# NIRVANALAN/LN3Diff

Measured on NVIDIA H100. Metric: denoised-latents/sec, higher is better.
Workload: dtype bf16

## Files before the change

ln3diff_b200/csrc/attention_wgmma.cu:

```cuda
#include <cstdlib>

#include "common.cuh"
#include "ln3_internal.h"

namespace ln3 {

static constexpr int kQT = 128;
static constexpr int kKT = 128;
static constexpr int kSW = 64;
static constexpr int kTileBytes = 128 * kSW * 2;
static constexpr int kStages = 4;
static constexpr int kThreads = 2 * 128 + 32;
static constexpr int kOrderBar = 1;
static constexpr int kTail = 8;
static constexpr int kTailBytes = 128 * kTail * 2;
static constexpr int kTailSmem = 2 * kTailBytes + kStages * 3 * kTailBytes;
template <int HD>
static constexpr int kFmhaSmem = 1024 + kTileBytes * (1 + 2 * kStages) + (HD > kSW ? kTailSmem : 0) + 256;

template <int HD>
struct FmhaTailMaps {
  CUtensorMap q, k, v;
};
template <>
struct FmhaTailMaps<64> {};

struct FmhaParams {
  int Lq, Lkv, Lkv2;
  int nb1, nb2;
  int H, n_qt;
  long long n_tiles;
  float scale_log2;
  int causal;
  __nv_bfloat16* out;
  long long o_ld, o_bs;
};

struct Tile {
  int q0, h, b, nb1, nblocks;
};

__device__ __forceinline__ Tile decode_tile(const FmhaParams& p, long long t) {
  Tile d;
  const long long bh = t / p.n_qt;
  d.q0 = static_cast<int>(t - bh * p.n_qt) * kQT;
  d.h = static_cast<int>(bh % p.H);
  d.b = static_cast<int>(bh / p.H);
  d.nb1 = p.causal ? min(p.nb1, (min(d.q0 + kQT, p.Lq) - 1) / kKT + 1) : p.nb1;
  d.nblocks = d.nb1 + p.nb2;
  return d;
}

__device__ __forceinline__ void softmax_block(const FmhaParams& p, float* s, float* m_run, float* l_run,
                                              float* alpha, int j, int nb1, int r0, int q) {
  const bool second = j >= nb1;
  const int kbase = (second ? j - nb1 : j) * kKT;
  const int klen = second ? p.Lkv2 : p.Lkv;
  const bool need_mask = kbase + kKT > klen || (p.causal && !second && kbase + kKT - 1 > r0);
  float mx[2] = {-INFINITY, -INFINITY};
#pragma unroll
  for (int i = 0; i < kKT / 8; ++i) {
#pragma unroll
    for (int e = 0; e < 4; ++e) {
      float v = __fmul_rn(s[4 * i + e], p.scale_log2);
      if (need_mask) {
        const int key = kbase + 8 * i + 2 * q + (e & 1);
        const int row = r0 + 8 * (e >> 1);
        if (key >= klen || (p.causal && !second && key > row)) v = -INFINITY;
      }
      s[4 * i + e] = v;
      mx[e >> 1] = fmaxf(mx[e >> 1], v);
    }
  }
  float m_use[2];
#pragma unroll
  for (int r = 0; r < 2; ++r) {
    mx[r] = fmaxf(mx[r], __shfl_xor_sync(0xffffffffu, mx[r], 1));
    mx[r] = fmaxf(mx[r], __shfl_xor_sync(0xffffffffu, mx[r], 2));
    const float m_new = fmaxf(m_run[r], mx[r]);
    m_use[r] = m_new == -INFINITY ? 0.f : m_new;
    alpha[r] = fast_exp2(__fsub_rn(m_run[r], m_use[r]));
    m_run[r] = m_new;
  }
#pragma unroll
  for (int kk = 0; kk < kKT / 16; ++kk) {
#pragma unroll
    for (int t = 0; t < 8; ++t) {
      const int r = (t >> 1) & 1;
      const float e = fast_exp2(__fsub_rn(s[8 * kk + t], m_use[r]));
      s[8 * kk + t] = e;
      l_run[r] = (kk == 0 && (t == 0 || t == 2)) ? __fmaf_rn(alpha[r], l_run[r], e) : __fadd_rn(l_run[r], e);
    }
  }
}

__device__ __forceinline__ void pack_p(const float* s, uint32_t (*pa)[4]) {
#pragma unroll
  for (int kk = 0; kk < kKT / 16; ++kk) {
    pa[kk][0] = pack_bf16x2(s[8 * kk + 0], s[8 * kk + 1]);
    pa[kk][1] = pack_bf16x2(s[8 * kk + 2], s[8 * kk + 3]);
    pa[kk][2] = pack_bf16x2(s[8 * kk + 4], s[8 * kk + 5]);
    pa[kk][3] = pack_bf16x2(s[8 * kk + 6], s[8 * kk + 7]);
  }
}

template <int HD>
__device__ __forceinline__ void issue_s(float* s, uint64_t q_desc, uint64_t k_desc, uint64_t qt_desc, uint64_t kt_desc) {
#pragma unroll
  for (int k = 0; k < kSW / 16; ++k) wgmma_m64n128k16_ss(s, q_desc + 2 * k, k_desc + 2 * k, k != 0 ? 1u : 0u);
  if constexpr (HD > kSW) wgmma_m64n128k16_ss(s, qt_desc, kt_desc, 1u);
  wgmma_commit();
}

template <int HD>
__device__ __forceinline__ void issue_pv(float* o, float* ot, const uint32_t (*pa)[4], uint64_t v_desc,
                                         uint64_t vt_desc) {
#pragma unroll
  for (int kk = 0; kk < kKT / 16; ++kk) {
    wgmma_m64n64k16_rs_tb(o, pa[kk], v_desc + kk * 128, 1u);
    if constexpr (HD > kSW) wgmma_m64n8k16_rs_tb(ot, pa[kk], vt_desc + kk * ((16 * kTail * 2) >> 4), 1u);
  }
  wgmma_commit();
}

template <int HD>
__global__ void __launch_bounds__(kThreads, 1)
fmha_fwd_kernel(const __grid_constant__ CUtensorMap tmap_q, const __grid_constant__ CUtensorMap tmap_k,
                const __grid_constant__ CUtensorMap tmap_v, const __grid_constant__ CUtensorMap tmap_k2,
                const __grid_constant__ CUtensorMap tmap_v2, const FmhaParams p,
                const __grid_constant__ FmhaTailMaps<HD> tails) {
  constexpr bool kHasTail = HD > kSW;
  extern __shared__ uint8_t smem_raw[];
  uint8_t* smem = reinterpret_cast<uint8_t*>((reinterpret_cast<uintptr_t>(smem_raw) + 1023) &
                                             ~static_cast<uintptr_t>(1023));
  uint8_t* sQ = smem;
  uint8_t* sK = sQ + kTileBytes;
  uint8_t* sV = sK + kStages * kTileBytes;
  uint8_t* sQt = sV + kStages * kTileBytes;
  uint8_t* sKt = sQt + 2 * kTailBytes;
  uint8_t* sVt = sKt + kStages * 2 * kTailBytes;
  uint64_t* bars = reinterpret_cast<uint64_t*>(sV + kStages * kTileBytes + (kHasTail ? kTailSmem : 0));
  uint64_t* q_full = bars;
  uint64_t* q_empty = bars + 1;
  uint64_t* kv_full = bars + 2;
  uint64_t* kv_empty = bars + 2 + kStages;

  const int warp = threadIdx.x >> 5;
  const int lane = threadIdx.x & 31;

  if (threadIdx.x == 0) {
    tma_prefetch_desc(&tmap_q);
    tma_prefetch_desc(&tmap_k);
    tma_prefetch_desc(&tmap_v);
    mbar_init(q_full, 1);
    mbar_init(q_empty, 2);
    for (int i = 0; i < kStages; ++i) {
      mbar_init(&kv_full[i], 1);
      mbar_init(&kv_empty[i], 2);
    }
    fence_barrier_init();
  }
  if constexpr (kHasTail) {
    for (int i = threadIdx.x; i < (1 + kStages) * (kTailBytes / 16); i += kThreads) {
      const int tile = i / (kTailBytes / 16), off = (i % (kTailBytes / 16)) * 16;
      *reinterpret_cast<uint4*>(sQt + tile * 2 * kTailBytes + kTailBytes + off) = make_uint4(0, 0, 0, 0);
    }
    fence_proxy_async_smem();
  }
  __syncthreads();

  if (warp == 8) {
    if (lane == 0) {
      int stage = 0;
      uint32_t phase = 0, tcount = 0;
      for (long long t = blockIdx.x; t < p.n_tiles; t += gridDim.x, ++tcount) {
        const Tile d = decode_tile(p, t);
        mbar_wait_silent(q_empty, (tcount & 1) ^ 1);
        mbar_arrive_expect_tx(q_full, kTileBytes + (kHasTail ? kTailBytes : 0));
        tma_load_3d(sQ, &tmap_q, q_full, d.h * HD, d.q0, d.b);
        if constexpr (kHasTail) tma_load_3d(sQt, &tails.q, q_full, d.h * HD + kSW, d.q0, d.b);
        for (int j = 0; j < d.nblocks; ++j) {
          mbar_wait_silent(&kv_empty[stage], phase ^ 1);
          mbar_arrive_expect_tx(&kv_full[stage], 2 * kTileBytes + (kHasTail ? 2 * kTailBytes : 0));
          const bool second = j >= d.nb1;
          const int row = (second ? j - d.nb1 : j) * kKT;
          tma_load_3d(sK + stage * kTileBytes, second ? &tmap_k2 : &tmap_k, &kv_full[stage], d.h * HD, row, d.b);
          tma_load_3d(sV + stage * kTileBytes, second ? &tmap_v2 : &tmap_v, &kv_full[stage], d.h * HD, row, d.b);
          if constexpr (kHasTail) {
            tma_load_3d(sKt + stage * 2 * kTailBytes, &tails.k, &kv_full[stage], d.h * HD + kSW, row, d.b);
            tma_load_3d(sVt + stage * kTailBytes, &tails.v, &kv_full[stage], d.h * HD + kSW, row, d.b);
          }
          if (++stage == kStages) {
            stage = 0;
            phase ^= 1;
          }
        }
      }
    }
    return;
  }

  const int wg = warp >> 2;
  const int g = lane >> 2, q = lane & 3;
  const bool leader = (threadIdx.x & 127) == 0;
  const uint64_t q_desc = make_smem_desc_sw128(smem_u32(sQ + wg * (64 * 128)), 16, 1024);
  const uint64_t k_desc0 = make_smem_desc_sw128(smem_u32(sK), 16, 1024);
  const uint64_t v_desc0 = make_smem_desc_sw128(smem_u32(sV), 16, 1024);
  const uint64_t qt_desc = make_smem_desc_plain(smem_u32(sQt + wg * 64 * (kTail * 2)), kTailBytes, 128);
  const uint64_t kt_desc0 = make_smem_desc_plain(smem_u32(sKt), kTailBytes, 128);
  const uint64_t vt_desc0 = make_smem_desc_plain(smem_u32(sVt), 128, 128);

  bool first_batch = true;
  auto batch_begin = [&]() {
    if (wg == 1 || !first_batch) named_bar_sync(kOrderBar + wg, 256);
    first_batch = false;
  };
  auto batch_end = [&](bool last) {
    if (wg == 0 || !last) named_bar_arrive(kOrderBar + (wg ^ 1), 256);
  };

  int stage = 0;
  uint32_t phase = 0, tcount = 0;
  for (long long t = blockIdx.x; t < p.n_tiles; t += gridDim.x, ++tcount) {
    const Tile d = decode_tile(p, t);
    const bool last_tile = t + gridDim.x >= p.n_tiles;
    const int r0 = d.q0 + wg * 64 + (warp & 3) * 16 + g;
    float o[kSW / 2], ot[4] = {0.f, 0.f, 0.f, 0.f};
#pragma unroll
    for (int i = 0; i < kSW / 2; ++i) o[i] = 0.f;
    float m_run[2] = {-INFINITY, -INFINITY}, l_run[2] = {0.f, 0.f}, alpha[2];
    float s[kKT / 2];
    uint32_t pa[kKT / 16][4];

    mbar_wait_silent(q_full, tcount & 1);
    mbar_wait_silent(&kv_full[stage], phase);
    batch_begin();
    wgmma_fence();
    issue_s<HD>(s, q_desc, k_desc0 + static_cast<uint32_t>(stage) * (kTileBytes >> 4), qt_desc,
                kt_desc0 + static_cast<uint32_t>(stage) * ((2 * kTailBytes) >> 4));
    batch_end(false);
    wgmma_wait<0>();
#pragma unroll
    for (int i = 0; i < kKT / 2; ++i) reg_fence(s[i]);
    if (d.nblocks == 1 && leader) mbar_arrive(q_empty);
    softmax_block(p, s, m_run, l_run, alpha, 0, d.nb1, r0, q);
    pack_p(s, pa);

    for (int j = 0; j + 1 < d.nblocks; ++j) {
      const int cur = stage;
      if (++stage == kStages) {
        stage = 0;
        phase ^= 1;
      }
      mbar_wait_silent(&kv_full[stage], phase);
      batch_begin();
      wgmma_fence();
      issue_s<HD>(s, q_desc, k_desc0 + static_cast<uint32_t>(stage) * (kTileBytes >> 4), qt_desc,
                  kt_desc0 + static_cast<uint32_t>(stage) * ((2 * kTailBytes) >> 4));
      issue_pv<HD>(o, ot, pa, v_desc0 + static_cast<uint32_t>(cur) * (kTileBytes >> 4),
                   vt_desc0 + static_cast<uint32_t>(cur) * (kTailBytes >> 4));
      batch_end(false);
      wgmma_wait<1>();
#pragma unroll
      for (int i = 0; i < kKT / 2; ++i) reg_fence(s[i]);
      if (j + 2 == d.nblocks && leader) mbar_arrive(q_empty);
      softmax_block(p, s, m_run, l_run, alpha, j + 1, d.nb1, r0, q);
      wgmma_wait<0>();
#pragma unroll
      for (int i = 0; i < kSW / 2; ++i) reg_fence(o[i]);
      if constexpr (kHasTail) {
#pragma unroll
        for (int i = 0; i < 4; ++i) reg_fence(ot[i]);
      }
      if (leader) mbar_arrive(&kv_empty[cur]);
#pragma unroll
      for (int i = 0; i < kSW / 8; ++i) {
        o[4 * i] *= alpha[0]; o[4 * i + 1] *= alpha[0];
        o[4 * i + 2] *= alpha[1]; o[4 * i + 3] *= alpha[1];
      }
      if constexpr (kHasTail) {
        ot[0] *= alpha[0]; ot[1] *= alpha[0];
        ot[2] *= alpha[1]; ot[3] *= alpha[1];
      }
      pack_p(s, pa);
    }

    batch_begin();
    wgmma_fence();
    issue_pv<HD>(o, ot, pa, v_desc0 + static_cast<uint32_t>(stage) * (kTileBytes >> 4),
                 vt_desc0 + static_cast<uint32_t>(stage) * (kTailBytes >> 4));
    batch_end(last_tile);
    wgmma_wait<0>();
#pragma unroll
    for (int i = 0; i < kSW / 2; ++i) reg_fence(o[i]);
    if constexpr (kHasTail) {
#pragma unroll
      for (int i = 0; i < 4; ++i) reg_fence(ot[i]);
    }
    if (leader) mbar_arrive(&kv_empty[stage]);
    if (++stage == kStages) {
      stage = 0;
      phase ^= 1;
    }

#pragma unroll
    for (int r = 0; r < 2; ++r) {
      l_run[r] += __shfl_xor_sync(0xffffffffu, l_run[r], 1);
      l_run[r] += __shfl_xor_sync(0xffffffffu, l_run[r], 2);
    }
    const float inv[2] = {l_run[0] > 0.f ? 1.f / l_run[0] : 0.f, l_run[1] > 0.f ? 1.f / l_run[1] : 0.f};
#pragma unroll
    for (int r = 0; r < 2; ++r) {
      const int row = r0 + 8 * r;
      if (row >= p.Lq) continue;
      __nv_bfloat16* dst = p.out + d.b * p.o_bs + row * p.o_ld + d.h * HD + 2 * q;
#pragma unroll
      for (int i = 0; i < kSW / 8; ++i)
        *reinterpret_cast<uint32_t*>(dst + 8 * i) =
            pack_bf16x2(o[4 * i + 2 * r] * inv[r], o[4 * i + 2 * r + 1] * inv[r]);
      if constexpr (kHasTail)
        *reinterpret_cast<uint32_t*>(dst + kSW) = pack_bf16x2(ot[2 * r] * inv[r], ot[2 * r + 1] * inv[r]);
    }
  }
}

template <int HD>
static int fmha_launch(const ln3_fmha_args* a, bool two, cudaStream_t stream) {
  static DeviceOnce once;
  if (int rc = once.run([] {
        cudaError_t e = cudaFuncSetAttribute(fmha_fwd_kernel<HD>, cudaFuncAttributeMaxDynamicSharedMemorySize,
                                             kFmhaSmem<HD>);
        return e == cudaSuccess ? LN3_OK : set_error(LN3_ECUDA, "fmha: cudaFuncSetAttribute: %s", cudaGetErrorString(e));
      }))
    return rc;
  CUtensorMap tq, tk, tv, tk2, tv2;
  FmhaTailMaps<HD> tails;
  int rc;
  const long long cols = static_cast<long long>(a->H) * HD;
  if ((rc = make_tmap_3d_bf16(&tq, a->q, cols, a->Lq, a->B, a->q_ld, a->q_bs, kSW, kQT))) return rc;
  if ((rc = make_tmap_3d_bf16(&tk, a->k, cols, a->Lkv, a->B, a->k_ld, a->k_bs, kSW, kKT))) return rc;
  if ((rc = make_tmap_3d_bf16(&tv, a->v, cols, a->Lkv, a->B, a->v_ld, a->v_bs, kSW, kKT))) return rc;
  if constexpr (HD > kSW) {
    if ((rc = make_tmap_3d_bf16(&tails.q, a->q, cols, a->Lq, a->B, a->q_ld, a->q_bs, kTail, kQT))) return rc;
    if ((rc = make_tmap_3d_bf16(&tails.k, a->k, cols, a->Lkv, a->B, a->k_ld, a->k_bs, kTail, kKT))) return rc;
    if ((rc = make_tmap_3d_bf16(&tails.v, a->v, cols, a->Lkv, a->B, a->v_ld, a->v_bs, kTail, kKT))) return rc;
  }
  if (two) {
    if ((rc = make_tmap_3d_bf16(&tk2, a->k2, cols, a->Lkv2, a->B, a->k2_ld, a->k2_bs, kSW, kKT))) return rc;
    if ((rc = make_tmap_3d_bf16(&tv2, a->v2, cols, a->Lkv2, a->B, a->v2_ld, a->v2_bs, kSW, kKT))) return rc;
  } else {
    tk2 = tk;
    tv2 = tv;
  }
  FmhaParams p;
  p.Lq = a->Lq;
  p.Lkv = a->Lkv;
  p.Lkv2 = two ? a->Lkv2 : 0;
  p.nb1 = (a->Lkv + kKT - 1) / kKT;
  p.nb2 = two ? (a->Lkv2 + kKT - 1) / kKT : 0;
  p.H = a->H;
  p.n_qt = (a->Lq + kQT - 1) / kQT;
  p.n_tiles = static_cast<long long>(p.n_qt) * a->H * a->B;
  p.scale_log2 = a->scale * 1.4426950408889634f;
  p.causal = a->causal ? 1 : 0;
  p.out = reinterpret_cast<__nv_bfloat16*>(a->out);
  p.o_ld = a->o_ld;
  p.o_bs = a->o_bs;
  const int sms = device_sm_count();
  const int grid = p.n_tiles < sms ? static_cast<int>(p.n_tiles) : sms;
  fmha_fwd_kernel<HD><<<grid, kThreads, kFmhaSmem<HD>, stream>>>(tq, tk, tv, tk2, tv2, p, tails);
  cudaError_t e = cudaGetLastError();
  if (e != cudaSuccess) return set_error(LN3_ECUDA, "fmha launch: %s", cudaGetErrorString(e));
  count_launch();
  return LN3_OK;
}

int fmha_fwd(const ln3_fmha_args* a, cudaStream_t stream) {
  if (a->head_dim != 64 && a->head_dim != 72) return set_error(LN3_EUNSUPPORTED, "fmha: head_dim must be 64 or 72");
  if (a->B <= 0 || a->H <= 0 || a->Lq <= 0 || a->Lkv <= 0)
    return set_error(LN3_EINVAL, "fmha: empty problem");
  if ((a->q_ld | a->k_ld | a->v_ld | a->o_ld | a->q_bs | a->k_bs | a->v_bs | a->o_bs) % 8)
    return set_error(LN3_EINVAL, "fmha: strides must be multiples of 8 elements");
  if ((reinterpret_cast<uintptr_t>(a->q) | reinterpret_cast<uintptr_t>(a->k) |
       reinterpret_cast<uintptr_t>(a->v) | reinterpret_cast<uintptr_t>(a->out)) & 15)
    return set_error(LN3_EINVAL, "fmha: pointers must be 16-byte aligned");
  if (a->causal && (a->k2 != nullptr || a->v2 != nullptr))
    return set_error(LN3_EINVAL, "fmha: causal attention takes a single K/V source");
  const bool two = a->k2 != nullptr || a->v2 != nullptr;
  if (two) {
    if (a->head_dim != 64) return set_error(LN3_EUNSUPPORTED, "fmha: a second K/V source needs head_dim 64");
    if (!a->k2 || !a->v2 || a->Lkv2 <= 0) return set_error(LN3_EINVAL, "fmha: k2/v2/Lkv2 must be given together");
    if ((a->k2_ld | a->v2_ld | a->k2_bs | a->v2_bs) % 8 ||
        ((reinterpret_cast<uintptr_t>(a->k2) | reinterpret_cast<uintptr_t>(a->v2)) & 15))
      return set_error(LN3_EINVAL, "fmha: k2/v2 alignment");
  }
  if (a->B > 65535 || a->H > 65535) return set_error(LN3_EUNSUPPORTED, "fmha: batch or head count above 65535");
  return a->head_dim == 64 ? fmha_launch<64>(a, two, stream) : fmha_launch<72>(a, two, stream);
}

}
```

Baseline: 1.389.

## Template FMHA on warpgroup count, add TMA output stores and register rebalancing

The attention kernel is now templated on the number of consumer warpgroups (2 or 3), so a Q tile can be 192 rows when that pads Lq less than 128-row tiles. A full producer warpgroup is added, and setmaxnreg shifts registers from the loader to the math warpgroups. Output now goes through a swizzled shared-memory staging buffer and TMA stores instead of direct per-thread global writes. The ordering barrier becomes a round-robin ring across warpgroups, and warpgroups whose rows fall past Lq skip their compute while still keeping barriers and pipeline stages in sync. This adds more shared memory and makes the synchronisation more complex.

```diff
diff --git a/ln3diff_b200/csrc/attention_wgmma.cu b/ln3diff_b200/csrc/attention_wgmma.cu
--- a/ln3diff_b200/csrc/attention_wgmma.cu
+++ b/ln3diff_b200/csrc/attention_wgmma.cu
@@ -5,22 +5,34 @@
 
 namespace ln3 {
 
-static constexpr int kQT = 128;
+static constexpr int kWGRows = 64;
 static constexpr int kKT = 128;
 static constexpr int kSW = 64;
-static constexpr int kTileBytes = 128 * kSW * 2;
+static constexpr int kKVBytes = kKT * kSW * 2;
+static constexpr int kWGBytes = kWGRows * kSW * 2;
 static constexpr int kStages = 4;
-static constexpr int kThreads = 2 * 128 + 32;
 static constexpr int kOrderBar = 1;
 static constexpr int kTail = 8;
-static constexpr int kTailBytes = 128 * kTail * 2;
-static constexpr int kTailSmem = 2 * kTailBytes + kStages * 3 * kTailBytes;
-template <int HD>
-static constexpr int kFmhaSmem = 1024 + kTileBytes * (1 + 2 * kStages) + (HD > kSW ? kTailSmem : 0) + 256;
+static constexpr int kKTailBytes = kKT * kTail * 2;
+
+template <int WG>
+struct FmhaTiles {
+  static constexpr int kQT = WG * kWGRows;
+  static constexpr int kQBytes = WG * kWGBytes;
+  static constexpr int kThreads = (WG + 1) * 128;
+  static constexpr int kMathRegs = WG == 3 ? 160 : 232, kLoadRegs = WG == 3 ? 32 : 40;
+  static_assert(WG * kMathRegs + kLoadRegs <= (WG + 1) * (65536 / kThreads / 8 * 8),
+                "the warpgroups' registers must fit the launch allocation");
+  static constexpr int kStoreBar = kOrderBar + WG;
+  static constexpr int kQTailBytes = kQT * kTail * 2;
+  static constexpr int kTailSmem = 3 * kQTailBytes + kStages * 3 * kKTailBytes;
+  template <int HD>
+  static constexpr int kSmem = 1024 + 2 * kQBytes + 2 * kStages * kKVBytes + (HD > kSW ? kTailSmem : 0) + 256;
+};
 
 template <int HD>
 struct FmhaTailMaps {
-  CUtensorMap q, k, v;
+  CUtensorMap q, k, v, o;
 };
 template <>
 struct FmhaTailMaps<64> {};
@@ -32,14 +44,13 @@
   long long n_tiles;
   float scale_log2;
   int causal;
-  __nv_bfloat16* out;
-  long long o_ld, o_bs;
 };
 
 struct Tile {
   int q0, h, b, nb1, nblocks;
 };
 
+template <int kQT>
 __device__ __forceinline__ Tile decode_tile(const FmhaParams& p, long long t) {
   Tile d;
   const long long bh = t / p.n_qt;
@@ -51,6 +62,10 @@
   return d;
 }
 
+__device__ __forceinline__ int wg_nb1(const FmhaParams& p, const Tile& d, int row0) {
+  return p.causal ? min(p.nb1, row0 / kKT + 1) : d.nb1;
+}
+
 __device__ __forceinline__ void softmax_block(const FmhaParams& p, float* s, float* m_run, float* l_run,
                                               float* alpha, int j, int nb1, int r0, int q) {
   const bool second = j >= nb1;
@@ -123,23 +138,27 @@
   wgmma_commit();
 }
 
-template <int HD>
-__global__ void __launch_bounds__(kThreads, 1)
+template <int HD, int kWG>
+__global__ void __launch_bounds__(FmhaTiles<kWG>::kThreads, 1)
 fmha_fwd_kernel(const __grid_constant__ CUtensorMap tmap_q, const __grid_constant__ CUtensorMap tmap_k,
                 const __grid_constant__ CUtensorMap tmap_v, const __grid_constant__ CUtensorMap tmap_k2,
-                const __grid_constant__ CUtensorMap tmap_v2, const FmhaParams p,
-                const __grid_constant__ FmhaTailMaps<HD> tails) {
+                const __grid_constant__ CUtensorMap tmap_v2, const __grid_constant__ CUtensorMap tmap_o,
+                const FmhaParams p, const __grid_constant__ FmhaTailMaps<HD> tails) {
   constexpr bool kHasTail = HD > kSW;
+  using T = FmhaTiles<kWG>;
+  constexpr int kQT = T::kQT, kQBytes = T::kQBytes, kThreads = T::kThreads, kQTailBytes = T::kQTailBytes;
   extern __shared__ uint8_t smem_raw[];
   uint8_t* smem = reinterpret_cast<uint8_t*>((reinterpret_cast<uintptr_t>(smem_raw) + 1023) &
                                              ~static_cast<uintptr_t>(1023));
   uint8_t* sQ = smem;
-  uint8_t* sK = sQ + kTileBytes;
-  uint8_t* sV = sK + kStages * kTileBytes;
-  uint8_t* sQt = sV + kStages * kTileBytes;
-  uint8_t* sKt = sQt + 2 * kTailBytes;
-  uint8_t* sVt = sKt + kStages * 2 * kTailBytes;
-  uint64_t* bars = reinterpret_cast<uint64_t*>(sV + kStages * kTileBytes + (kHasTail ? kTailSmem : 0));
+  uint8_t* sK = sQ + kQBytes;
+  uint8_t* sV = sK + kStages * kKVBytes;
+  uint8_t* sO = sV + kStages * kKVBytes;
+  uint8_t* sQt = sO + kQBytes;
+  uint8_t* sKt = sQt + 2 * kQTailBytes;
+  uint8_t* sVt = sKt + kStages * 2 * kKTailBytes;
+  uint8_t* sOt = sVt + kStages * kKTailBytes;
+  uint64_t* bars = reinterpret_cast<uint64_t*>(sO + kQBytes + (kHasTail ? T::kTailSmem : 0));
   uint64_t* q_full = bars;
   uint64_t* q_empty = bars + 1;
   uint64_t* kv_full = bars + 2;
@@ -152,43 +171,196 @@
     tma_prefetch_desc(&tmap_q);
     tma_prefetch_desc(&tmap_k);
     tma_prefetch_desc(&tmap_v);
+    tma_prefetch_desc(&tmap_o);
     mbar_init(q_full, 1);
-    mbar_init(q_empty, 2);
+    mbar_init(q_empty, kWG);
     for (int i = 0; i < kStages; ++i) {
       mbar_init(&kv_full[i], 1);
-      mbar_init(&kv_empty[i], 2);
+      mbar_init(&kv_empty[i], kWG);
     }
     fence_barrier_init();
   }
   if constexpr (kHasTail) {
-    for (int i = threadIdx.x; i < (1 + kStages) * (kTailBytes / 16); i += kThreads) {
-      const int tile = i / (kTailBytes / 16), off = (i % (kTailBytes / 16)) * 16;
-      *reinterpret_cast<uint4*>(sQt + tile * 2 * kTailBytes + kTailBytes + off) = make_uint4(0, 0, 0, 0);
+    for (int i = threadIdx.x; i < kQTailBytes / 16; i += kThreads)
+      *reinterpret_cast<uint4*>(sQt + kQTailBytes + 16 * i) = make_uint4(0, 0, 0, 0);
+    for (int i = threadIdx.x; i < kStages * (kKTailBytes / 16); i += kThreads) {
+      const int tile = i / (kKTailBytes / 16), off = (i % (kKTailBytes / 16)) * 16;
+      *reinterpret_cast<uint4*>(sKt + tile * 2 * kKTailBytes + kKTailBytes + off) = make_uint4(0, 0, 0, 0);
     }
     fence_proxy_async_smem();
   }
   __syncthreads();
 
-  if (warp == 8) {
-    if (lane == 0) {
+  if (warp < 4 * kWG) {
+    setmaxnreg_inc<T::kMathRegs>();
+
+    const int wg = warp >> 2;
+    const int g = lane >> 2, q = lane & 3;
+    const bool leader = (threadIdx.x & 127) == 0;
+    const uint64_t q_desc = make_smem_desc_sw128(smem_u32(sQ + wg * kWGBytes), 16, 1024);
+    const uint64_t k_desc0 = make_smem_desc_sw128(smem_u32(sK), 16, 1024);
+    const uint64_t v_desc0 = make_smem_desc_sw128(smem_u32(sV), 16, 1024);
+    const uint64_t qt_desc = make_smem_desc_plain(smem_u32(sQt + wg * kWGRows * (kTail * 2)), kQTailBytes, 128);
+    const uint64_t kt_desc0 = make_smem_desc_plain(smem_u32(sKt), kKTailBytes, 128);
+    const uint64_t vt_desc0 = make_smem_desc_plain(smem_u32(sVt), 128, 128);
+
+    if (wg == kWG - 1) named_bar_arrive(kOrderBar, 256);
+    auto turn_begin = [&]() { named_bar_sync(kOrderBar + wg, 256); };
+    auto turn_end = [&](bool last) {
+      if (wg != kWG - 1 || !last) named_bar_arrive(kOrderBar + (wg + 1) % kWG, 256);
+    };
+
+    uint32_t kv = 0;
+    for (uint32_t tcount = 0;; ++tcount) {
+      const long long t = blockIdx.x + static_cast<long long>(tcount) * gridDim.x;
+      if (t >= p.n_tiles) break;
+      const Tile d = decode_tile<kQT>(p, t);
+      const bool last_tile = t + gridDim.x >= p.n_tiles;
+      const int row0 = d.q0 + wg * kWGRows;
+      const int nb1 = wg_nb1(p, d, row0);
+      const int nbw = row0 < p.Lq ? nb1 + (kHasTail ? 0 : p.nb2) : 0;
+      float o[kSW / 2], ot[4] = {0.f, 0.f, 0.f, 0.f};
+#pragma unroll
+      for (int i = 0; i < kSW / 2; ++i) o[i] = 0.f;
+      float m_run[2] = {-INFINITY, -INFINITY}, l_run[2] = {0.f, 0.f}, alpha[2];
+      float s[kKT / 2];
+      uint32_t pa[kKT / 16][4];
+      int k0 = 0;
+      if (nbw > 0) {
+        const int r0 = row0 + (warp & 3) * 16 + g;
+
+        mbar_wait_silent(q_full, tcount & 1);
+        mbar_wait_silent(&kv_full[kv % kStages], (kv / kStages) & 1);
+        turn_begin();
+        wgmma_fence();
+        issue_s<HD>(s, q_desc, k_desc0 + (kv % kStages) * (kKVBytes >> 4), qt_desc,
+                    kt_desc0 + (kv % kStages) * ((2 * kKTailBytes) >> 4));
+        turn_end(false);
+        wgmma_wait<0>();
+#pragma unroll
+        for (int i = 0; i < kKT / 2; ++i) reg_fence(s[i]);
+        if (nbw == 1 && leader) mbar_arrive(q_empty);
+        softmax_block(p, s, m_run, l_run, alpha, 0, nb1, r0, q);
+        pack_p(s, pa);
+
+        for (int j = 0; j + 1 < nbw; ++j) {
+          const uint32_t cur = kv % kStages;
+          ++kv;
+          mbar_wait_silent(&kv_full[kv % kStages], (kv / kStages) & 1);
+          turn_begin();
+          wgmma_fence();
+          issue_s<HD>(s, q_desc, k_desc0 + (kv % kStages) * (kKVBytes >> 4), qt_desc,
+                      kt_desc0 + (kv % kStages) * ((2 * kKTailBytes) >> 4));
+          issue_pv<HD>(o, ot, pa, v_desc0 + cur * (kKVBytes >> 4),
+                       vt_desc0 + cur * (kKTailBytes >> 4));
+          turn_end(false);
+          wgmma_wait<1>();
+#pragma unroll
+          for (int i = 0; i < kKT / 2; ++i) reg_fence(s[i]);
+          if (j + 2 == nbw && leader) mbar_arrive(q_empty);
+          softmax_block(p, s, m_run, l_run, alpha, j + 1, nb1, r0, q);
+          wgmma_wait<0>();
+#pragma unroll
+          for (int i = 0; i < kSW / 2; ++i) reg_fence(o[i]);
+          if constexpr (kHasTail) {
+#pragma unroll
+            for (int i = 0; i < 4; ++i) reg_fence(ot[i]);
+          }
+          if (leader) mbar_arrive(&kv_empty[cur]);
+#pragma unroll
+          for (int i = 0; i < kSW / 8; ++i) {
+            o[4 * i] *= alpha[0]; o[4 * i + 1] *= alpha[0];
+            o[4 * i + 2] *= alpha[1]; o[4 * i + 3] *= alpha[1];
+          }
+          if constexpr (kHasTail) {
+            ot[0] *= alpha[0]; ot[1] *= alpha[0];
+            ot[2] *= alpha[1]; ot[3] *= alpha[1];
+          }
+          pack_p(s, pa);
+        }
+
+        turn_begin();
+        wgmma_fence();
+        issue_pv<HD>(o, ot, pa, v_desc0 + (kv % kStages) * (kKVBytes >> 4),
+                     vt_desc0 + (kv % kStages) * (kKTailBytes >> 4));
+        turn_end(last_tile && nbw == d.nblocks);
+        wgmma_wait<0>();
+#pragma unroll
+        for (int i = 0; i < kSW / 2; ++i) reg_fence(o[i]);
+        if constexpr (kHasTail) {
+#pragma unroll
+          for (int i = 0; i < 4; ++i) reg_fence(ot[i]);
+        }
+        if (leader) mbar_arrive(&kv_empty[kv % kStages]);
+        ++kv;
+        k0 = nbw + 1;
+      } else {
+        mbar_wait_silent(q_full, tcount & 1);
+        if (leader) mbar_arrive(q_empty);
+      }
+      for (int k = k0; k <= d.nblocks; ++k) {
+        turn_begin();
+        turn_end(last_tile && k == d.nblocks);
+        if (k == 0) continue;
+        mbar_wait_silent(&kv_full[kv % kStages], (kv / kStages) & 1);
+        if (leader) mbar_arrive(&kv_empty[kv % kStages]);
+        ++kv;
+      }
+
+      if (nbw > 0) {
+#pragma unroll
+        for (int r = 0; r < 2; ++r) {
+          l_run[r] += __shfl_xor_sync(0xffffffffu, l_run[r], 1);
+          l_run[r] += __shfl_xor_sync(0xffffffffu, l_run[r], 2);
+        }
+        const float inv[2] = {l_run[0] > 0.f ? 1.f / l_run[0] : 0.f, l_run[1] > 0.f ? 1.f / l_run[1] : 0.f};
+        if (leader) tma_store_wait_read();
+        named_bar_sync(T::kStoreBar + wg, 128);
+        uint8_t* const sOw = sO + wg * kWGBytes;
+        uint8_t* const sOtw = sOt + wg * kWGRows * (kTail * 2);
+#pragma unroll
+        for (int r = 0; r < 2; ++r) {
+          const int row = (warp & 3) * 16 + g + 8 * r;
+          uint8_t* line = sOw + row * (kSW * 2);
+#pragma unroll
+          for (int i = 0; i < kSW / 8; ++i)
+            *reinterpret_cast<uint32_t*>(line + ((i ^ (row & 7)) << 4) + 4 * q) =
+                pack_bf16x2(o[4 * i + 2 * r] * inv[r], o[4 * i + 2 * r + 1] * inv[r]);
+          if constexpr (kHasTail)
+            *reinterpret_cast<uint32_t*>(sOtw + row * (kTail * 2) + 4 * q) =
+                pack_bf16x2(ot[2 * r] * inv[r], ot[2 * r + 1] * inv[r]);
+        }
+        fence_proxy_async_smem();
+        named_bar_sync(T::kStoreBar + wg, 128);
+        if (leader) {
+          tma_store_3d(sOw, &tmap_o, d.h * HD, row0, d.b);
+          if constexpr (kHasTail) tma_store_3d(sOtw, &tails.o, d.h * HD + kSW, row0, d.b);
+          tma_store_commit();
+        }
+      }
+    }
+    if (leader) tma_store_wait_all();
+  } else {
+    setmaxnreg_dec<T::kLoadRegs>();
+    if (warp == 4 * kWG && lane == 0) {
       int stage = 0;
       uint32_t phase = 0, tcount = 0;
       for (long long t = blockIdx.x; t < p.n_tiles; t += gridDim.x, ++tcount) {
-        const Tile d = decode_tile(p, t);
+        const Tile d = decode_tile<kQT>(p, t);
         mbar_wait_silent(q_empty, (tcount & 1) ^ 1);
-        mbar_arrive_expect_tx(q_full, kTileBytes + (kHasTail ? kTailBytes : 0));
+        mbar_arrive_expect_tx(q_full, kQBytes + (kHasTail ? kQTailBytes : 0));
         tma_load_3d(sQ, &tmap_q, q_full, d.h * HD, d.q0, d.b);
         if constexpr (kHasTail) tma_load_3d(sQt, &tails.q, q_full, d.h * HD + kSW, d.q0, d.b);
         for (int j = 0; j < d.nblocks; ++j) {
           mbar_wait_silent(&kv_empty[stage], phase ^ 1);
-          mbar_arrive_expect_tx(&kv_full[stage], 2 * kTileBytes + (kHasTail ? 2 * kTailBytes : 0));
+          mbar_arrive_expect_tx(&kv_full[stage], 2 * kKVBytes + (kHasTail ? 2 * kKTailBytes : 0));
           const bool second = j >= d.nb1;
           const int row = (second ? j - d.nb1 : j) * kKT;
-          tma_load_3d(sK + stage * kTileBytes, second ? &tmap_k2 : &tmap_k, &kv_full[stage], d.h * HD, row, d.b);
-          tma_load_3d(sV + stage * kTileBytes, second ? &tmap_v2 : &tmap_v, &kv_full[stage], d.h * HD, row, d.b);
+          tma_load_3d(sK + stage * kKVBytes, second ? &tmap_k2 : &tmap_k, &kv_full[stage], d.h * HD, row, d.b);
+          tma_load_3d(sV + stage * kKVBytes, second ? &tmap_v2 : &tmap_v, &kv_full[stage], d.h * HD, row, d.b);
           if constexpr (kHasTail) {
-            tma_load_3d(sKt + stage * 2 * kTailBytes, &tails.k, &kv_full[stage], d.h * HD + kSW, row, d.b);
-            tma_load_3d(sVt + stage * kTailBytes, &tails.v, &kv_full[stage], d.h * HD + kSW, row, d.b);
+            tma_load_3d(sKt + stage * 2 * kKTailBytes, &tails.k, &kv_full[stage], d.h * HD + kSW, row, d.b);
+            tma_load_3d(sVt + stage * kKTailBytes, &tails.v, &kv_full[stage], d.h * HD + kSW, row, d.b);
           }
           if (++stage == kStages) {
             stage = 0;
@@ -197,153 +369,33 @@
         }
       }
     }
-    return;
-  }
-
-  const int wg = warp >> 2;
-  const int g = lane >> 2, q = lane & 3;
-  const bool leader = (threadIdx.x & 127) == 0;
-  const uint64_t q_desc = make_smem_desc_sw128(smem_u32(sQ + wg * (64 * 128)), 16, 1024);
-  const uint64_t k_desc0 = make_smem_desc_sw128(smem_u32(sK), 16, 1024);
-  const uint64_t v_desc0 = make_smem_desc_sw128(smem_u32(sV), 16, 1024);
-  const uint64_t qt_desc = make_smem_desc_plain(smem_u32(sQt + wg * 64 * (kTail * 2)), kTailBytes, 128);
-  const uint64_t kt_desc0 = make_smem_desc_plain(smem_u32(sKt), kTailBytes, 128);
-  const uint64_t vt_desc0 = make_smem_desc_plain(smem_u32(sVt), 128, 128);
-
-  bool first_batch = true;
-  auto batch_begin = [&]() {
-    if (wg == 1 || !first_batch) named_bar_sync(kOrderBar + wg, 256);
-    first_batch = false;
-  };
-  auto batch_end = [&](bool last) {
-    if (wg == 0 || !last) named_bar_arrive(kOrderBar + (wg ^ 1), 256);
-  };
-
-  int stage = 0;
-  uint32_t phase = 0, tcount = 0;
-  for (long long t = blockIdx.x; t < p.n_tiles; t += gridDim.x, ++tcount) {
-    const Tile d = decode_tile(p, t);
-    const bool last_tile = t + gridDim.x >= p.n_tiles;
-    const int r0 = d.q0 + wg * 64 + (warp & 3) * 16 + g;
-    float o[kSW / 2], ot[4] = {0.f, 0.f, 0.f, 0.f};
-#pragma unroll
-    for (int i = 0; i < kSW / 2; ++i) o[i] = 0.f;
-    float m_run[2] = {-INFINITY, -INFINITY}, l_run[2] = {0.f, 0.f}, alpha[2];
-    float s[kKT / 2];
-    uint32_t pa[kKT / 16][4];
-
-    mbar_wait_silent(q_full, tcount & 1);
-    mbar_wait_silent(&kv_full[stage], phase);
-    batch_begin();
-    wgmma_fence();
-    issue_s<HD>(s, q_desc, k_desc0 + static_cast<uint32_t>(stage) * (kTileBytes >> 4), qt_desc,
-                kt_desc0 + static_cast<uint32_t>(stage) * ((2 * kTailBytes) >> 4));
-    batch_end(false);
-    wgmma_wait<0>();
-#pragma unroll
-    for (int i = 0; i < kKT / 2; ++i) reg_fence(s[i]);
-    if (d.nblocks == 1 && leader) mbar_arrive(q_empty);
-    softmax_block(p, s, m_run, l_run, alpha, 0, d.nb1, r0, q);
-    pack_p(s, pa);
-
-    for (int j = 0; j + 1 < d.nblocks; ++j) {
-      const int cur = stage;
-      if (++stage == kStages) {
-        stage = 0;
-        phase ^= 1;
-      }
-      mbar_wait_silent(&kv_full[stage], phase);
-      batch_begin();
-      wgmma_fence();
-      issue_s<HD>(s, q_desc, k_desc0 + static_cast<uint32_t>(stage) * (kTileBytes >> 4), qt_desc,
-                  kt_desc0 + static_cast<uint32_t>(stage) * ((2 * kTailBytes) >> 4));
-      issue_pv<HD>(o, ot, pa, v_desc0 + static_cast<uint32_t>(cur) * (kTileBytes >> 4),
-                   vt_desc0 + static_cast<uint32_t>(cur) * (kTailBytes >> 4));
-      batch_end(false);
-      wgmma_wait<1>();
-#pragma unroll
-      for (int i = 0; i < kKT / 2; ++i) reg_fence(s[i]);
-      if (j + 2 == d.nblocks && leader) mbar_arrive(q_empty);
-      softmax_block(p, s, m_run, l_run, alpha, j + 1, d.nb1, r0, q);
-      wgmma_wait<0>();
-#pragma unroll
-      for (int i = 0; i < kSW / 2; ++i) reg_fence(o[i]);
-      if constexpr (kHasTail) {
-#pragma unroll
-        for (int i = 0; i < 4; ++i) reg_fence(ot[i]);
-      }
-      if (leader) mbar_arrive(&kv_empty[cur]);
-#pragma unroll
-      for (int i = 0; i < kSW / 8; ++i) {
-        o[4 * i] *= alpha[0]; o[4 * i + 1] *= alpha[0];
-        o[4 * i + 2] *= alpha[1]; o[4 * i + 3] *= alpha[1];
-      }
-      if constexpr (kHasTail) {
-        ot[0] *= alpha[0]; ot[1] *= alpha[0];
-        ot[2] *= alpha[1]; ot[3] *= alpha[1];
-      }
-      pack_p(s, pa);
-    }
-
-    batch_begin();
-    wgmma_fence();
-    issue_pv<HD>(o, ot, pa, v_desc0 + static_cast<uint32_t>(stage) * (kTileBytes >> 4),
-                 vt_desc0 + static_cast<uint32_t>(stage) * (kTailBytes >> 4));
-    batch_end(last_tile);
-    wgmma_wait<0>();
-#pragma unroll
-    for (int i = 0; i < kSW / 2; ++i) reg_fence(o[i]);
-    if constexpr (kHasTail) {
-#pragma unroll
-      for (int i = 0; i < 4; ++i) reg_fence(ot[i]);
-    }
-    if (leader) mbar_arrive(&kv_empty[stage]);
-    if (++stage == kStages) {
-      stage = 0;
-      phase ^= 1;
-    }
-
-#pragma unroll
-    for (int r = 0; r < 2; ++r) {
-      l_run[r] += __shfl_xor_sync(0xffffffffu, l_run[r], 1);
-      l_run[r] += __shfl_xor_sync(0xffffffffu, l_run[r], 2);
-    }
-    const float inv[2] = {l_run[0] > 0.f ? 1.f / l_run[0] : 0.f, l_run[1] > 0.f ? 1.f / l_run[1] : 0.f};
-#pragma unroll
-    for (int r = 0; r < 2; ++r) {
-      const int row = r0 + 8 * r;
-      if (row >= p.Lq) continue;
-      __nv_bfloat16* dst = p.out + d.b * p.o_bs + row * p.o_ld + d.h * HD + 2 * q;
-#pragma unroll
-      for (int i = 0; i < kSW / 8; ++i)
-        *reinterpret_cast<uint32_t*>(dst + 8 * i) =
-            pack_bf16x2(o[4 * i + 2 * r] * inv[r], o[4 * i + 2 * r + 1] * inv[r]);
-      if constexpr (kHasTail)
-        *reinterpret_cast<uint32_t*>(dst + kSW) = pack_bf16x2(ot[2 * r] * inv[r], ot[2 * r + 1] * inv[r]);
-    }
-  }
-}
-
-template <int HD>
+  }
+}
+
+template <int HD, int kWG>
 static int fmha_launch(const ln3_fmha_args* a, bool two, cudaStream_t stream) {
+  using T = FmhaTiles<kWG>;
+  constexpr int kQT = T::kQT;
   static DeviceOnce once;
   if (int rc = once.run([] {
-        cudaError_t e = cudaFuncSetAttribute(fmha_fwd_kernel<HD>, cudaFuncAttributeMaxDynamicSharedMemorySize,
-                                             kFmhaSmem<HD>);
+        cudaError_t e = cudaFuncSetAttribute(fmha_fwd_kernel<HD, kWG>, cudaFuncAttributeMaxDynamicSharedMemorySize,
+                                             T::template kSmem<HD>);
         return e == cudaSuccess ? LN3_OK : set_error(LN3_ECUDA, "fmha: cudaFuncSetAttribute: %s", cudaGetErrorString(e));
       }))
     return rc;
-  CUtensorMap tq, tk, tv, tk2, tv2;
+  CUtensorMap tq, tk, tv, tk2, tv2, to;
   FmhaTailMaps<HD> tails;
   int rc;
   const long long cols = static_cast<long long>(a->H) * HD;
   if ((rc = make_tmap_3d_bf16(&tq, a->q, cols, a->Lq, a->B, a->q_ld, a->q_bs, kSW, kQT))) return rc;
   if ((rc = make_tmap_3d_bf16(&tk, a->k, cols, a->Lkv, a->B, a->k_ld, a->k_bs, kSW, kKT))) return rc;
   if ((rc = make_tmap_3d_bf16(&tv, a->v, cols, a->Lkv, a->B, a->v_ld, a->v_bs, kSW, kKT))) return rc;
+  if ((rc = make_tmap_3d_bf16(&to, a->out, cols, a->Lq, a->B, a->o_ld, a->o_bs, kSW, kWGRows))) return rc;
   if constexpr (HD > kSW) {
     if ((rc = make_tmap_3d_bf16(&tails.q, a->q, cols, a->Lq, a->B, a->q_ld, a->q_bs, kTail, kQT))) return rc;
     if ((rc = make_tmap_3d_bf16(&tails.k, a->k, cols, a->Lkv, a->B, a->k_ld, a->k_bs, kTail, kKT))) return rc;
     if ((rc = make_tmap_3d_bf16(&tails.v, a->v, cols, a->Lkv, a->B, a->v_ld, a->v_bs, kTail, kKT))) return rc;
+    if ((rc = make_tmap_3d_bf16(&tails.o, a->out, cols, a->Lq, a->B, a->o_ld, a->o_bs, kTail, kWGRows))) return rc;
   }
   if (two) {
     if ((rc = make_tmap_3d_bf16(&tk2, a->k2, cols, a->Lkv2, a->B, a->k2_ld, a->k2_bs, kSW, kKT))) return rc;
@@ -363,12 +415,9 @@
   p.n_tiles = static_cast<long long>(p.n_qt) * a->H * a->B;
   p.scale_log2 = a->scale * 1.4426950408889634f;
   p.causal = a->causal ? 1 : 0;
-  p.out = reinterpret_cast<__nv_bfloat16*>(a->out);
-  p.o_ld = a->o_ld;
-  p.o_bs = a->o_bs;
   const int sms = device_sm_count();
   const int grid = p.n_tiles < sms ? static_cast<int>(p.n_tiles) : sms;
-  fmha_fwd_kernel<HD><<<grid, kThreads, kFmhaSmem<HD>, stream>>>(tq, tk, tv, tk2, tv2, p, tails);
+  fmha_fwd_kernel<HD, kWG><<<grid, T::kThreads, T::template kSmem<HD>, stream>>>(tq, tk, tv, tk2, tv2, to, p, tails);
   cudaError_t e = cudaGetLastError();
   if (e != cudaSuccess) return set_error(LN3_ECUDA, "fmha launch: %s", cudaGetErrorString(e));
   count_launch();
@@ -395,7 +444,9 @@
       return set_error(LN3_EINVAL, "fmha: k2/v2 alignment");
   }
   if (a->B > 65535 || a->H > 65535) return set_error(LN3_EUNSUPPORTED, "fmha: batch or head count above 65535");
-  return a->head_dim == 64 ? fmha_launch<64>(a, two, stream) : fmha_launch<72>(a, two, stream);
-}
-
-}
+  const bool rows128 = (a->Lq + 127) / 128 * 128 < (a->Lq + 191) / 192 * 192;
+  if (a->head_dim == 64) return rows128 ? fmha_launch<64, 2>(a, two, stream) : fmha_launch<64, 3>(a, two, stream);
+  return rows128 ? fmha_launch<72, 2>(a, two, stream) : fmha_launch<72, 3>(a, two, stream);
+}
+
+}
```

After: 1.432 (median of 6 runs). 1.03x the previous value.
